# DEEPDIP-project/IncompressibleNavierStokes.jl

Measured on AMD Instinct MI355X. Metric: M lattice-cell updates/sec (RK4 step incl. Poisson), 3D TGV fp64, higher is better.
Workload: dtype f64; 1 GPU; TaylorGreenVortex3D 256^3 periodic fp64, RK44 + spectral Poisson, dt=0.001, Re=1e3; decomposition=single GPU, loop=timesteps_ (K steps, one native call)

## Files before the change

incompressiblenavierstokes.jl_amd/csrc/ins_flux128.hip:

```cpp
#include <algorithm>
#include <cstring>

#include "ins_internal.h"
#include "ins_wave64.h"
#include "ins_flux_common.h"

namespace {

template <typename T>
struct P2 {
  T a, b;
};
template <typename T>
__device__ __forceinline__ P2<T> ldb2(rsrc_t r, unsigned voff, unsigned soff);
template <>
__device__ __forceinline__ P2<double> ldb2<double>(rsrc_t r, unsigned voff, unsigned soff) {
  const v4u v = __builtin_amdgcn_raw_buffer_load_b128(r, voff, soff, 0);
  return {__hiloint2double((int)v.y, (int)v.x), __hiloint2double((int)v.w, (int)v.z)};
}
template <>
__device__ __forceinline__ P2<float> ldb2<float>(rsrc_t r, unsigned voff, unsigned soff) {
  const v2u v = __builtin_amdgcn_raw_buffer_load_b64(r, voff, soff, 0);
  return {__int_as_float((int)v.x), __int_as_float((int)v.y)};
}
// ... 6 lines not shown
  __builtin_amdgcn_raw_buffer_store_b128(v, r, voff, soff, 0);
}
__device__ __forceinline__ void stb2(rsrc_t r, unsigned voff, unsigned soff, float a, float b) {
  v2u v;
  v.x = (unsigned)__float_as_int(a);
  v.y = (unsigned)__float_as_int(b);
  __builtin_amdgcn_raw_buffer_store_b64(v, r, voff, soff, 0);
}

template <typename T, int R>
struct Plane2 {
  P2<T> v[3][R + 2];
  T h[3];
};

template <typename T, int R, int XW, bool FUSE, int CORR, int NW>
__global__ __launch_bounds__(64 * NW, (CORR && R == 2 && NW == 4 && sizeof(T) == 8) ? 1 : 2) void k_flux128(FluxArgs a) {
  constexpr unsigned EB = (unsigned)sizeof(T);
  constexpr int WC = 128;
  const T* const a_u = static_cast<const T*>(a.u);
  const T* const a_pI = static_cast<const T*>(a.pI);
  T* const a_F = static_cast<T*>(a.F);
  static_assert(R + 3 <= 8, "packed halo rows live in 8-lane groups");
  int txi, tyi, tzi;
  {
    const int nty_local = (a.nty + 7) >> 3;
    int seq = (int)(blockIdx.x >> 3);
    if (seq >= a.ntx * nty_local * a.ntz) return;
    txi = seq % a.ntx;
    seq /= a.ntx;
    tyi = (int)(blockIdx.x & 7) * nty_local + seq % nty_local;
    tzi = seq / nty_local;
// ... 87 lines not shown
      const T Wn = next_h(Wa, rdlane(C.h[2], 16 + rr));
      zprev[0][rr - 1].a = flux(C.v[0][rr].a, Nx.v[0][rr].a, Wa, Wb, Z.vo);
      zprev[0][rr - 1].b = flux(C.v[0][rr].b, Nx.v[0][rr].b, Wb, Wn, Z.vo);
      zprev[1][rr - 1].a = flux(C.v[1][rr].a, Nx.v[1][rr].a, Wa, C.v[2][rr + 1].a, Z.vo);
      zprev[1][rr - 1].b = flux(C.v[1][rr].b, Nx.v[1][rr].b, Wb, C.v[2][rr + 1].b, Z.vo);
      zprev[2][rr - 1].a = flux(Wa, Nx.v[2][rr].a, Wa, Nx.v[2][rr].a, Z.vs);
      zprev[2][rr - 1].b = flux(Wb, Nx.v[2][rr].b, Wb, Nx.v[2][rr].b, Z.vs);
    }
  };

  unsigned orow[R];
#pragma unroll
  for (int rr = 0; rr < R; ++rr) orow[rr] = (unsigned)((min(jb0 + rr, n1 - 1) + 1) * N0) * EB;
  const unsigned ocol = ucol;

  auto epi_load = [&](const Plane2<T, R>& C, int k, P2<T> (&sacc)[3][R]) {
    const long long pk = (long long)k * sz;
    if (a.epi.ustart) {
      const T* b = static_cast<const T*>((const void*)a.epi.ustart) + pk;
      const T c0 = (T)(1.0 + a.epi.c0m1);
#pragma unroll
      for (int c = 0; c < 3; ++c) {
        const rsrc_t rs = plane_rsrc(b + c * a.sc, ubytes);
#pragma unroll
        for (int rr = 0; rr < R; ++rr) {
          const P2<T> v = ldb2<T>(rs, ocol, orow[rr]);
          sacc[c][rr].a = c0 * v.a;
          sacc[c][rr].b = c0 * v.b;
        }
      }
    } else {
#pragma unroll
      for (int c = 0; c < 3; ++c)
#pragma unroll
        for (int rr = 0; rr < R; ++rr) sacc[c][rr] = C.v[c][rr + 1];
    }
    if (a.epi.self_in != 0.0) {
      const T cs = (T)a.epi.self_in;
      if (CORR) {
        const T* b = a_u + (long long)uplane(k) * sz;
#pragma unroll
// ... 21 lines not shown
      const T cq = (T)a.epi.coef[q];
#pragma unroll
      for (int c = 0; c < 3; ++c) {
        const rsrc_t rs = plane_rsrc(kq + c * a.sc, ubytes);
        P2<T> kv[R];
#pragma unroll
        for (int rr = 0; rr < R; ++rr) kv[rr] = ldb2<T>(rs, ocol, orow[rr]);
#pragma unroll
        for (int rr = 0; rr < R; ++rr) {
          sacc[c][rr].a += cq * kv[rr].a;
          sacc[c][rr].b += cq * kv[rr].b;
        }
      }
    }
  };
  auto emit = [&](int rr, int k, const P2<T>& fu, const P2<T>& fv, const P2<T>& fw, const P2<T>& s0, const P2<T>& s1, const P2<T>& s2) {
    const long long pk = (long long)k * sz;
    const int j = jb0 + rr - 1;
    if (xout && j < n1) {
      const unsigned rowb = orow[rr - 1], co = ocol;
      if (FUSE) {
        if (CORR && a.epi.ustart_out) {
          T* w = static_cast<T*>((void*)a.epi.ustart_out) + pk;
          stb2(plane_rsrc(w, ubytes), co, rowb, s0.a, s0.b);
          stb2(plane_rsrc(w + a.sc, ubytes), co, rowb, s1.a, s1.b);
          stb2(plane_rsrc(w + 2 * a.sc, ubytes), co, rowb, s2.a, s2.b);
        }
        T* o = static_cast<T*>((void*)a.epi.ustar) + pk;
        const T cs = (T)a.epi.coef_self;
        stb2(plane_rsrc(o, ubytes), co, rowb, s0.a + cs * fu.a, s0.b + cs * fu.b);
        stb2(plane_rsrc(o + a.sc, ubytes), co, rowb, s1.a + cs * fv.a, s1.b + cs * fv.b);
        stb2(plane_rsrc(o + 2 * a.sc, ubytes), co, rowb, s2.a + cs * fw.a, s2.b + cs * fw.b);
      }
      if (!FUSE || a.epi.write_k) {
        T* o = a_F + pk;
        stb2(plane_rsrc(o, ubytes), co, rowb, fu.a, fu.b);
        stb2(plane_rsrc(o + a.sc, ubytes), co, rowb, fv.a, fv.b);
        stb2(plane_rsrc(o + 2 * a.sc, ubytes), co, rowb, fw.a, fw.b);
      }
    }
  };

  auto body = [&](Plane2<T, R>& C, const Plane2<T, R>& Nx, int k, int kload) {
    const T* nb = a_u + (long long)uplane(kload) * sz;
    const rsrc_t n0r = plane_rsrc(nb, ubytes), n1r = plane_rsrc(nb + a.sc, ubytes), n2r = plane_rsrc(nb + 2 * a.sc, ubytes);
    const T ch0 = C.h[0], ch1 = C.h[1], ch2 = C.h[2];
    P2<T> sacc[3][FUSE ? R : 1];
    if constexpr (FUSE) epi_load(C, k, sacc);
    P2<T> fyu_o = {0, 0}, fyv_o = {0, 0}, fyw_o = {0, 0};
#pragma unroll
    for (int rr = 0; rr <= R; ++rr) {
      const T Ua = C.v[0][rr].a, Ub = C.v[0][rr].b, Va = C.v[1][rr].a, Vb = C.v[1][rr].b, Wa = C.v[2][rr].a, Wb = C.v[2][rr].b;
      const T Vn = next_h(Va, rdlane(ch1, 16 + rr));
      P2<T> fyu, fyv, fyw;
      fyu.a = flux(Ua, C.v[0][rr + 1].a, Va, Vb, Y.vo);
      fyu.b = flux(Ub, C.v[0][rr + 1].b, Vb, Vn, Y.vo);
      fyv.a = flux(Va, C.v[1][rr + 1].a, Va, C.v[1][rr + 1].a, Y.vs);
      fyv.b = flux(Vb, C.v[1][rr + 1].b, Vb, C.v[1][rr + 1].b, Y.vs);
      fyw.a = flux(Wa, C.v[2][rr + 1].a, Va, Nx.v[1][rr].a, Y.vo);
      fyw.b = flux(Wb, C.v[2][rr + 1].b, Vb, Nx.v[1][rr].b, Y.vo);
      if (rr >= 1) {
        const T Un = next_h(Ua, rdlane(ch0, 16 + rr)), Wn = next_h(Wa, rdlane(ch2, 16 + rr));
        const T fxu_a = flux(Ua, Ub, Ua, Ub, X.vs), fxu_b = flux(Ub, Un, Ub, Un, X.vs);
// ... 21 lines not shown
        zu.a = flux(Ua, Nx.v[0][rr].a, Wa, Wb, Z.vo);
        zu.b = flux(Ub, Nx.v[0][rr].b, Wb, Wn, Z.vo);
        zv.a = flux(Va, Nx.v[1][rr].a, Wa, C.v[2][rr + 1].a, Z.vo);
        zv.b = flux(Vb, Nx.v[1][rr].b, Wb, C.v[2][rr + 1].b, Z.vo);
        zw.a = flux(Wa, Nx.v[2][rr].a, Wa, Nx.v[2][rr].a, Z.vs);
        zw.b = flux(Wb, Nx.v[2][rr].b, Wb, Nx.v[2][rr].b, Z.vs);
        fu.a += (zu.a - zprev[0][rr - 1].a) * Z.ro;
        fu.b += (zu.b - zprev[0][rr - 1].b) * Z.ro;
        fv.a += (zv.a - zprev[1][rr - 1].a) * Z.ro;
        fv.b += (zv.b - zprev[1][rr - 1].b) * Z.ro;
        fw.a += (zw.a - zprev[2][rr - 1].a) * Z.rs;
        fw.b += (zw.b - zprev[2][rr - 1].b) * Z.rs;
        zprev[0][rr - 1] = zu;
        zprev[1][rr - 1] = zv;
        zprev[2][rr - 1] = zw;
        if constexpr (FUSE)
          emit(rr, k, fu, fv, fw, sacc[0][rr - 1], sacc[1][rr - 1], sacc[2][rr - 1]);
        else
          emit(rr, k, fu, fv, fw, fu, fu, fu);
      }
      fyu_o = fyu;
      fyv_o = fyv;
      fyw_o = fyw;
      C.v[0][rr] = ldb2<T>(n0r, ucol, urow[rr]);
      C.v[1][rr] = ldb2<T>(n1r, ucol, urow[rr]);
      C.v[2][rr] = ldb2<T>(n2r, ucol, urow[rr]);
    }
    C.v[0][R + 1] = ldb2<T>(n0r, ucol, urow[R + 1]);
    C.v[1][R + 1] = ldb2<T>(n1r, ucol, urow[R + 1]);
    C.v[2][R + 1] = ldb2<T>(n2r, ucol, urow[R + 1]);
    C.h[0] = ldb<T>(n0r, uhoff, 0);
// ... 38 lines not shown
      if (++k >= k1) break;
      if (a.bar) __builtin_amdgcn_s_barrier();
      correct(P1, Pb, Hb, Pa, Ha);
      load_p(Pb, Hb, min(k + 3, k1 + 1));
      body(P0, P1, k, min(k + 2, k1));
      if (++k >= k1) break;
    }
  }
}

template <typename T, int R, int XW, bool FUSE, int NW>
int launch_range(FluxArgs& a, int corr_mode, hipStream_t s) {
  const unsigned nb = (unsigned)(8LL * a.ntx * ((a.nty + 7) / 8) * a.ntz);
  if (nb == 0) return INS_OK;
  const dim3 block(64, NW, 1);
  if (corr_mode == 0)
    hipLaunchKernelGGL((k_flux128<T, R, XW, FUSE, 0, NW>), dim3(nb), block, 0, s, a);
  else if constexpr (FUSE) {
    if (corr_mode == 1)
      hipLaunchKernelGGL((k_flux128<T, R, XW, true, 1, NW>), dim3(nb), block, 0, s, a);
    else
      hipLaunchKernelGGL((k_flux128<T, R, XW, true, 2, NW>), dim3(nb), block, 0, s, a);
  } else {
    ins_set_error("in-kernel pressure correction needs the fused epilogue");
    return INS_ERR_UNSUPPORTED;
  }
  INS_LAUNCH_CHECK();
  return INS_OK;
}

// ... 118 lines not shown
```

incompressiblenavierstokes.jl_amd/csrc/ins_flux64.hip:

```cpp
#include <algorithm>
#include <cstdlib>
#include <cstring>

#include "ins_internal.h"
#include "ins_wave64.h"
#include "ins_flux_common.h"

namespace {

template <typename T, int R>
struct Plane {
  T v[3][R + 2];
  T h[3];
  T raw[3][R];
};

template <typename T, int R>
struct TExt {
  T t[R + 2];
  T th;
  T vm1;
};

template <typename T, int R, int XW, bool FUSE, int CORR, bool SKEL = false, int NW = 4, bool EXTRA = false>
__global__ __launch_bounds__(64 * NW, NW == 16 ? 4 : 2) void k_flux64(FluxArgs a) {
  constexpr unsigned EB = (unsigned)sizeof(T);
  const T* const a_u = static_cast<const T*>(a.u);
  const T* const a_pI = static_cast<const T*>(a.pI);
  T* const a_F = static_cast<T*>(a.F);
  static_assert(R + 2 + (CORR ? 1 : 0) <= 8, "packed halo rows live in 8-lane groups");
  int txi, tyi, tzi;
  {
    const int nty_local = (a.nty + 7) >> 3;
    int seq = (int)(blockIdx.x >> 3);
    if (seq >= a.ntx * nty_local * a.ntz) return;
    txi = seq % a.ntx;
    seq /= a.ntx;
    tyi = (int)(blockIdx.x & 7) * nty_local + seq % nty_local;
    tzi = seq / nty_local;
    if (tyi >= a.nty) return;
// ... 61 lines not shown
  auto load_text = [&](TExt<T, R>& E, int kk) {
    const long long po = (long long)uplane(kk) * sz;
    const rsrc_t rt = plane_rsrc(static_cast<const T*>((const void*)a.te.temp) + po, ubytes);
#pragma unroll
    for (int rr = 0; rr < R + 2; ++rr) E.t[rr] = ldb<T>(rt, ucol, urow[rr]);
    E.th = ldb<T>(rt, uhoff, 0);
    E.vm1 = ldb<T>(plane_rsrc(a_u + po + a.sc, ubytes), ucol, urowm1);
  };
  auto load_p = [&](T (&P)[R + 3], T& PH, int kk) {
    const rsrc_t rs = plane_rsrc(a_pI + (long long)(CORR == 2 ? min(kk, N2) : wrapi(kk - 1, n2)) * n0 * n1, qbytes);
#pragma unroll
    for (int rr = 0; rr < R + 3; ++rr) P[rr] = ldb<T>(rs, qcol, qrow[rr]);
    PH = ldb<T>(rs, qhoff, 0);
  };
  auto correct = [&](Plane<T, R>& P, const T (&Pc)[R + 3], T PHc, const T (&Pn)[R + 3], T PHn) {
    if (a.epi.self_in != 0.0) {
#pragma unroll
      for (int c = 0; c < 3; ++c)
#pragma unroll
        for (int rr = 0; rr < R; ++rr) P.raw[c][rr] = P.v[c][rr + 1];
    }
#pragma unroll
    for (int rr = 0; rr < R + 2; ++rr) {
      const T pc = Pc[rr];
      P.v[0][rr] -= (next_h(pc, rdlane(PHc, 16 + rr)) - pc) * X.gs;
      P.v[1][rr] -= (Pc[rr + 1] - pc) * Y.gs;
      P.v[2][rr] -= (Pn[rr] - pc) * Z.gs;
    }
    P.h[0] -= (dpp_old<0x108>(PHc, PHc) - PHc) * X.gs;
    P.h[1] -= (dpp_old<0x101>(PHc, PHc) - PHc) * Y.gs;
    P.h[2] -= (PHn - PHc) * Z.gs;
// ... 7 lines not shown
      zprev[0][rr - 1] = flux(C.v[0][rr], Nx.v[0][rr], Wc, next_h(Wc, rdlane(C.h[2], 16 + rr)), Z.vo);
      zprev[1][rr - 1] = flux(C.v[1][rr], Nx.v[1][rr], Wc, C.v[2][rr + 1], Z.vo);
      zprev[2][rr - 1] = flux(Wc, Nx.v[2][rr], Wc, Nx.v[2][rr], Z.vs);
    }
  };

  unsigned orow[R];
#pragma unroll
  for (int rr = 0; rr < R; ++rr) orow[rr] = (unsigned)((min(jb0 + rr, n1 - 1) + 1) * N0) * EB;
  const unsigned ocol = (unsigned)(min(ci, n0 - 1) + 1) * EB;

  T eacc[3][EXTRA ? R : 1];
  T gacc[EXTRA ? R : 1];
  T Pz[3][EXTRA ? R : 1];
  const T nux = X.vs * X.rs, nuy = Y.vs * Y.rs, nuz = Z.vs * Z.rs;
  auto epi_load = [&](const Plane<T, R>& C, int k, T (&sacc)[3][R]) {
    const long long pk = (long long)k * sz;
    if constexpr (EXTRA) {
      if (a.epi.extra) {
        const T* b = static_cast<const T*>((const void*)a.epi.extra) + pk;
#pragma unroll
        for (int c = 0; c < 3; ++c) {
          const rsrc_t rs = plane_rsrc(b + c * a.sc, ubytes);
#pragma unroll
          for (int rr = 0; rr < R; ++rr) eacc[c][rr] = ldb<T>(rs, ocol, orow[rr]);
        }
      } else {
#pragma unroll
        for (int c = 0; c < 3; ++c)
#pragma unroll
          for (int rr = 0; rr < R; ++rr) eacc[c][rr] = 0;
// ... 3 lines not shown
        const int gd = a.epi.gdir;
        const rsrc_t r0 = plane_rsrc(tb, ubytes), r1 = plane_rsrc(gd == 2 ? tb + sz : tb, ubytes);
        const unsigned dcol = gd == 0 ? EB : 0u, drow = gd == 1 ? (unsigned)N0 * EB : 0u;
#pragma unroll
        for (int rr = 0; rr < R; ++rr) gacc[rr] = (T)a.epi.ga2 * ((T)0.5 * (ldb<T>(r0, ocol, orow[rr]) + ldb<T>(r1, ocol + dcol, orow[rr] + drow)));
      }
    }
    const bool ntl = (a.nt & 8) != 0;
    if (a.epi.ustart) {
      const T* b = static_cast<const T*>((const void*)a.epi.ustart) + pk;
      const T c0 = (T)(1.0 + a.epi.c0m1);
#pragma unroll
      for (int c = 0; c < 3; ++c) {
        const rsrc_t rs = plane_rsrc(b + c * a.sc, ubytes);
#pragma unroll
        for (int rr = 0; rr < R; ++rr) sacc[c][rr] = c0 * (ntl ? ldb_aux<2>(rs, ocol, orow[rr], (T)0) : ldb<T>(rs, ocol, orow[rr]));
      }
    } else {
#pragma unroll
      for (int c = 0; c < 3; ++c)
#pragma unroll
        for (int rr = 0; rr < R; ++rr) sacc[c][rr] = C.v[c][rr + 1];
    }
    if (a.epi.self_in != 0.0) {
#pragma unroll
      for (int c = 0; c < 3; ++c)
#pragma unroll
        for (int rr = 0; rr < R; ++rr) sacc[c][rr] += (T)a.epi.self_in * (CORR ? C.raw[c][rr] : C.v[c][rr + 1]);
    }
    for (int q = 0; q < a.epi.n; ++q) {
      const T* kq = static_cast<const T*>((const void*)a.epi.k[q]) + pk;
// ... 18 lines not shown
      stb(r2, co, rowb, v2);
    } else if (snt == 1) {
      stb_aux<2>(r0, co, rowb, v0);
      stb_aux<2>(r1, co, rowb, v1);
      stb_aux<2>(r2, co, rowb, v2);
    } else if (snt == 2) {
      stb_aux<17>(r0, co, rowb, v0);
      stb_aux<17>(r1, co, rowb, v1);
      stb_aux<17>(r2, co, rowb, v2);
    } else {
      stb_aux<19>(r0, co, rowb, v0);
      stb_aux<19>(r1, co, rowb, v1);
      stb_aux<19>(r2, co, rowb, v2);
    }
  };
  auto emit = [&](int rr, int k, T fu, T fv, T fw, T s0, T s1, T s2) {
    const long long pk = (long long)k * sz;
    if constexpr (EXTRA) {
      fu += eacc[0][rr - 1];
      fv += eacc[1][rr - 1];
      fw += eacc[2][rr - 1];
      if (a.epi.gtemp) {
        const T gv = gacc[rr - 1];
        if (a.epi.gdir == 0) fu += gv;
        if (a.epi.gdir == 1) fv += gv;
        if (a.epi.gdir == 2) fw += gv;
      }
    }
    const int j = jb0 + rr - 1;
    if (xout && j < n1) {
      const unsigned rowb = orow[rr - 1], co = ocol;
      if (FUSE) {
        if (CORR && a.epi.ustart_out) {
          T* w = static_cast<T*>((void*)a.epi.ustart_out) + pk;
          stb(plane_rsrc(w, ubytes), co, rowb, s0);
          stb(plane_rsrc(w + a.sc, ubytes), co, rowb, s1);
          stb(plane_rsrc(w + 2 * a.sc, ubytes), co, rowb, s2);
        }
        T* o = static_cast<T*>((void*)a.epi.ustar) + pk;
        st3(o, co, rowb, s0 + (T)a.epi.coef_self * fu, s1 + (T)a.epi.coef_self * fv, s2 + (T)a.epi.coef_self * fw);
      }
      if (!FUSE || a.epi.write_k) st3(a_F + pk, co, rowb, fu, fv, fw);
    }
  };

  constexpr bool TMK = EXTRA && CORR == 0;
  T Tz[TMK ? R : 1];
  T wwprev[TMK ? R : 1];
  T PzV0 = 0;
  T hU_prev = 0;
  auto body = [&](Plane<T, R>& C, const Plane<T, R>& Nx, TExt<T, R>& CT, const TExt<T, R>& NT, int k, int kload) {
    const T* nb = a_u + (long long)uplane(kload) * sz;
    const rsrc_t n0r = plane_rsrc(nb, ubytes), n1r = plane_rsrc(nb + a.sc, ubytes), n2r = plane_rsrc(nb + 2 * a.sc, ubytes);
    const T ch0 = C.h[0], ch1 = C.h[1], ch2 = C.h[2];
    T sacc[3][R];
    if (FUSE) epi_load(C, k, sacc);
    const bool tm = TMK && a.tm;
    const rsrc_t ntr = plane_rsrc(static_cast<const T*>((const void*)a.te.temp) + (long long)uplane(kload) * sz, ubytes);
    T tacc[TMK ? R : 1];
    const T cth = CT.th;
    if constexpr (TMK) {
      if (tm) {
        const long long pk = (long long)k * sz;
        const rsrc_t rs0 = plane_rsrc(static_cast<const T*>((const void*)a.te.tempstart) + pk, ubytes);
#pragma unroll
        for (int rr = 0; rr < R; ++rr) tacc[rr] = ldb<T>(rs0, ocol, orow[rr]);
        for (int q = 0; q < a.te.n; ++q) {
          const rsrc_t rq = plane_rsrc(static_cast<const T*>((const void*)a.te.k[q]) + pk, ubytes);
#pragma unroll
          for (int rr = 0; rr < R; ++rr) tacc[rr] += (T)a.te.coef[q] * ldb<T>(rq, ocol, orow[rr]);
        }
// ... 80 lines not shown
              const T kt = cd + dd;
              if (xout && j < n1) {
                const long long pk = (long long)k * sz;
                if (a.te.ktemp_out) stb(plane_rsrc(static_cast<T*>((void*)a.te.ktemp_out) + pk, ubytes), ocol, orow[rr - 1], kt);
                stb(plane_rsrc(static_cast<T*>((void*)a.te.temp_out) + pk, ubytes), ocol, orow[rr - 1], tacc[rr - 1] + (T)a.te.c_self * kt);
              }
              wv_o = wv;
              wwprev[rr - 1] = ww;
              Tz[rr - 1] = Tc;
            }
          }
          Pz[0][rr - 1] = Uc;
          Pz[1][rr - 1] = Vc;
          Pz[2][rr - 1] = Wc;
        }
        emit(rr, k, fu, fv, fw, FUSE ? sacc[0][rr - 1] : (T)0, FUSE ? sacc[1][rr - 1] : (T)0, FUSE ? sacc[2][rr - 1] : (T)0);
      }
      fyu_o = fyu;
      fyv_o = fyv;
      fyw_o = fyw;
      if constexpr (TMK) {
        if (tm) {
          if (rr == 0) {
            const T Vp = prev_h(Vc, rdlane(ch1, 0));
            wv_o = jb0 > 0 ? Vc * ((Vn + Vp - 2 * Vc) * nux + (C.v[1][1] + CT.vm1 - 2 * Vc) * nuy + (Nx.v[1][0] + PzV0 - 2 * Vc) * nuz) : (T)0;
            PzV0 = Vc;
          }
          To = CT.t[rr];
          CT.t[rr] = ldb<T>(ntr, ucol, urow[rr]);
        }
      }
// ... 104 lines not shown
#define g_lds ((int)ins_opt(OPT_INS_FLUX64_LDS))
#define g_skel ((int)ins_opt(OPT_INS_FLUX64_SKEL))

template <typename T, int R, int XW, bool FUSE, int NW>
int launch_range(const ins_grid* G, FluxArgs& a, int corr_mode, hipStream_t s) {
  const unsigned nb = (unsigned)(8LL * a.ntx * ((a.nty + 7) / 8) * a.ntz);
  if (nb == 0) return INS_OK;
  const dim3 block(64, NW, 1);
  if constexpr (NW <= 8 && R == 4 && sizeof(T) == 8) {
    if (g_skel && corr_mode == 0) {
      hipLaunchKernelGGL((k_flux64<T, R, XW, FUSE, 0, true, NW>), dim3(nb), block, (size_t)g_lds, s, a);
      INS_LAUNCH_CHECK();
      return INS_OK;
    }
  }
  if (a.tm && corr_mode != 0) {
    ins_set_error("temperature stage inside the stage kernel: no in-kernel pressure correction");
    return INS_ERR_UNSUPPORTED;
  }
  if (a.epi.extra || a.epi.gtemp || a.epi.wout || a.tm) {
    if constexpr (FUSE && R == 2 && NW == 4 && sizeof(T) == 8) {
      if (corr_mode == 0) {
        hipLaunchKernelGGL((k_flux64<T, R, XW, true, 0, false, NW, true>), dim3(nb), block, (size_t)g_lds, s, a);
        INS_LAUNCH_CHECK();
        return INS_OK;
      }
      if (corr_mode == 1) {
        hipLaunchKernelGGL((k_flux64<T, R, XW, true, 1, false, NW, true>), dim3(nb), block, (size_t)g_lds, s, a);
        INS_LAUNCH_CHECK();
        return INS_OK;
// ... 46 lines not shown

extern "C" void ins_tune_flux64(int disable, int rows, int rows_corr, int zchunk, int xw, int skel, int burst_unused, int lds) {
  if (disable >= 0) ins_set_option("INS_DISABLE_FLUX64", disable);
  if (rows >= 0) ins_set_option("INS_FLUX64_ROWS", rows);
  if (rows_corr >= 0) ins_set_option("INS_FLUX64_ROWS_CORR", rows_corr);
  if (zchunk >= 0) ins_set_option("INS_FLUX64_ZC", zchunk);
  if (xw >= 0) ins_set_option("INS_FLUX64_XW", xw);
  if (skel >= 0) ins_set_option("INS_FLUX64_SKEL", skel);
  (void)burst_unused;
  if (lds >= 0) ins_set_option("INS_FLUX64_LDS", lds);
}

bool ins_flux64_supported(const ins_grid* G) {
  const GridDev& g = G->g;
  return !g_disable && g.D == 3 && G->all_dof && G->uniform_exact && g.N[0] - 2 >= 66 && g.N[1] - 2 >= 8 && g.N[2] - 2 >= 4;
}

template <typename T>
static int flux64_dispatch(const ins_grid* G, double visc, const T* u, T* F, const RkEpi* epi, const T* pI, int corr_mode, hipStream_t s, int part) {
  const GridDev& g = G->g;
  FluxArgs a;
  memset(&a, 0, sizeof(a));
  a.u = u;
  a.pI = pI;
  a.F = F;
  a.sc = g.sc;
  a.N0 = g.N[0];
  a.N1 = g.N[1];
  a.N2 = g.N[2];
  const int n2 = g.N[2] - 2;
// ... 109 lines not shown
```

incompressiblenavierstokes.jl_amd/csrc/ins_flux_common.h:

```cpp
#pragma once
#include "ins_internal.h"

namespace {

struct Dir {
  double vs, vo;
  double rs, ro;
  double gs;
};
template <typename T>
struct DirT {
  T vs, vo, rs, ro, gs;
  __device__ DirT(const Dir& d) : vs((T)d.vs), vo((T)d.vo), rs((T)d.rs), ro((T)d.ro), gs((T)d.gs) {}
};

struct FluxArgs {
  const void* u;
  const void* pI;
  void* F;
  long long sc;
  int N0, N1, N2;
  int zc, ntx, nty, ntz;
  int k_lo, k_hi, kB;
  int nt;
  int bar;
  Dir X, Y, Z;
  RkEpi epi;
  int tm;
  TempEpi te;
};

template <typename T>
__device__ __forceinline__ T flux(T uc, T up, T ub0, T ub1, T vd4) {
  return (up - uc) * vd4 - (uc + up) * (ub0 + ub1);
}

static Dir make_dir(const ins_grid* G, int d, double visc) {
  const double dxu = G->desc.dxu[d][1], dx1 = G->desc.dx[d][1], dx2 = G->desc.dx[d][2];
  Dir r;
  r.vs = 4.0 * (visc * (dx2 > 2 * INS_EPS ? 1.0 / dx2 : 0.0));
  r.vo = 4.0 * (visc * (dxu > 2 * INS_EPS ? 1.0 / dxu : 0.0));
  r.gs = 1.0 / dxu;
  r.rs = 0.25 * r.gs;
  r.ro = 0.25 * (1.0 / dx1);
  return r;
}

}
```

incompressiblenavierstokes.jl_amd/csrc/ins_internal.h:

```cpp
#pragma once

#include <hip/hip_runtime.h>
#include <hipfft/hipfft.h>

#include <cstdint>
#include <cstdio>
#include <cstring>
#include <string>
#include <vector>

#include "ins_hip.h"

#define INS_EPS 2.220446049250313e-16
#define INS_MAX_STAGES 16

void ins_set_error(const char* fmt, ...);

#define INS_HIP_TRY(expr)                                                                   \
  do {                                                                                      \
    hipError_t _e = (expr);                                                                 \
    if (_e != hipSuccess) {                                                                 \
      ins_set_error("%s:%d: %s -> %s", __FILE__, __LINE__, #expr, hipGetErrorString(_e));   \
      return INS_ERR_HIP;                                                                   \
    }                                                                                       \
// ... 69 lines not shown
  X(INS_FLUX64_LDS)              \
  X(INS_FLUX64_SKEL)             \
  X(INS_FLUX64_NW)               \
  X(INS_FLUX64_NT)               \
  X(INS_FLUX64_NOBAR)            \
  X(INS_FLUX64_MINTILES)         \
  X(INS_FLUX64_XW_CORR)          \
  X(INS_UNIFORM_BITWISE)         \
  X(INS_PHAT_DENSE)              \
  X(INS_DISABLE_FDM_FUSED)       \
  X(INS_DISABLE_FDM_FOLD)        \
  X(INS_DISABLE_FDM_UNFOLD4)     \
  X(INS_DISABLE_FDM_FOLDFUSE)    \
  X(INS_DISABLE_INKERNEL_CORR)   \
  X(INS_RK_KEEP_K)               \
  X(INS_DISABLE_EXT_FUSED)       \
  X(INS_EXT_TEMP_SPLIT)          \
  X(INS_DISABLE_FUSED_RK)        \
  X(INS_DISABLE_STEP_CHAIN)      \
  X(INS_DISABLE_STEP_GRAPH)      \
  X(INS_DISABLE_LINE3)           \
  X(INS_DISABLE_XYFUSED)         \
  X(INS_DISABLE_CORR2D)          \
  X(INS_SPECTRUM_ROCFFT)         \
  X(INS_X_SKEL)                  \
  X(INS_LINE3_TK)                \
  X(INS_LINE3_WGS)               \
  X(INS_STEP_GRAPH)              \
  X(INS_ZSOLVE_SKEL)             \
  X(INS_ZSOLVE_TK)               \
// ... 141 lines not shown
struct Rec {
  double vs, vo, a0, b0, a1, b1, a2, b2, rs, ro, pad[6];
};

struct RkEpi {
  int n;
  int write_k;
  double coef[INS_MAX_STAGES + 1];
  const double* k[INS_MAX_STAGES + 1];
  double coef_self;
  double self_in;
  double c0m1;
  const double* ustart;
  double* ustar;
  double* ustart_out;
  const double* extra;
  const double* gtemp;
  double ga2;
  int gdir;
  double* wout;
  const struct TempEpi* tstage;
};

struct TempEpi {
  const double* temp;
  const double* tempstart;
  double* temp_out;
  double* ktemp_out;
  int n;
  double coef[INS_MAX_STAGES];
// ... 90 lines not shown
```

incompressiblenavierstokes.jl_amd/csrc/ins_rk.hip:

```cpp
#include <cstdlib>

#include "ins_internal.h"


int ins_k_momentum_generic(const ins_grid* G, double visc, const double* u, double* F, hipStream_t s);
int ins_k_momentum_fast3d(const ins_grid* G, double visc, const double* u, double* F, hipStream_t s);
int ins_k_momentum_fast3d_opts(const ins_grid* G, double visc, const double* u, double* F, bool zero_shell, hipStream_t s);
bool ins_fast3d_supported(const ins_grid* G);
bool ins_flux64_supported(const ins_grid* G);

int ins_k_momentum_rk_fused(const ins_grid* G, double visc, const double* u_in, double* k_out, const RkEpi& epi, hipStream_t s);
int ins_k_project_periodic_fused(const ins_grid* G, ins_poisson* ps, double* u, double* p, bool keep_p, hipStream_t s, double* uout = nullptr);

int ins_k_momentum(const ins_grid* G, double visc, const double* u, double* F, hipStream_t s) {
  if (ins_fast3d_supported(G)) return ins_k_momentum_fast3d(G, visc, u, F, s);
  return ins_k_momentum_generic(G, visc, u, F, s);
}

namespace {

struct Combine {
  int n;
  double coef[INS_MAX_STAGES + 1];
  const double* k[INS_MAX_STAGES + 1];
// ... 37 lines not shown
static int combine_n(long long nvec, const double* base, double* out, int nterms, const double* coefs, const double* const* ks, void* stream) {
  INS_REQUIRE(nterms >= 0 && nterms <= INS_MAX_STAGES + 1 && (nterms == 0 || (coefs && ks)), "bad stage terms");
  Combine cb;
  cb.n = 0;
  for (int q = 0; q < nterms; ++q) {
    if (coefs[q] == 0.0) continue;
    INS_REQUIRE(ks[q], "null stage field");
    cb.coef[cb.n] = coefs[q];
    cb.k[cb.n] = ks[q];
    ++cb.n;
  }
  const unsigned nblk = (unsigned)std::min<long long>((nvec / 2 + 255) / 256, 8192);
  hipLaunchKernelGGL(k_combine, dim3(nblk), dim3(256), 0, as_stream(stream), nvec, base, out, cb);
  INS_LAUNCH_CHECK();
  return INS_OK;
}

static void step_graph_free(ins_rk* rk);
bool ins_k_spectral_own3d(const ins_poisson* ps);

extern "C" int ins_rk_create(const ins_grid_t* G, ins_poisson_t* ps, int nstage, const double* A, const double* c, ins_rk_t** out) {
  INS_REQUIRE(G && ps && A && c && out, "null argument");
  INS_REQUIRE(ps->grid == G, "psolver was created for a different grid");
  INS_REQUIRE(nstage >= 1 && nstage <= INS_MAX_STAGES, "unsupported number of stages");
  for (int i = 0; i < nstage; ++i)
    for (int j = i + 1; j < nstage; ++j) INS_REQUIRE(A[i * nstage + j] == 0.0, "shifted tableau must be lower triangular (explicit method)");
  ins_rk* rk = new ins_rk();
  rk->grid = G;
  rk->ps = ps;
  rk->nstage = nstage;
// ... 78 lines not shown
  const int ns = rk->nstage;
  const size_t vbytes = (size_t)G->ncell * 3 * sizeof(double);
  for (int b = 0; b < 2; ++b)
    if (!rk->ub[b]) {
      INS_HIP_TRY(hipMalloc(&rk->ub[b], vbytes));
      INS_HIP_TRY(hipMemsetAsync(rk->ub[b], 0, vbytes, s));
    }
  int rc;
  const bool raw_in = chain & 1, raw_out = chain & 2;
  if (!raw_in && (rc = ins_k_apply_bc_u(G, u, 0, nullptr, s))) return rc;
  const bool no_corr = ins_opt(OPT_INS_DISABLE_INKERNEL_CORR) != 0;
  const bool inkernel = !no_corr && G->uniform_exact && ns > 1 && G->g.N[0] >= 8 && G->g.N[1] >= 8 && G->g.N[2] >= 8;
  const bool keep_k = ins_opt(OPT_INS_RK_KEEP_K) != 0;
  bool vbasis = inkernel && !keep_k;
  for (int i = 0; vbasis && i < ns; ++i) vbasis = rk->A[i * ns + i] != 0.0;
  if (vbasis && (int)rk->vb.size() < ns - 1) {
    rk->vb.resize(ns - 1, nullptr);
    for (int m = 0; m < ns - 1; ++m)
      if (!rk->vb[m]) {
        if (m < 2 && rk->ub[m]) {
          rk->vb[m] = rk->ub[m];
          continue;
        }
        INS_HIP_TRY(hipMalloc(&rk->vb[m], vbytes));
        INS_HIP_TRY(hipMemsetAsync(rk->vb[m], 0, vbytes, s));
      }
  }
  const double* in = u;
  for (int i = 0; i < ns; ++i) {
    double* out = (i == ns - 1 && ns > 1) ? u : (vbasis ? rk->vb[i] : rk->ub[i & 1]);
    RkEpi epi;
    memset(&epi, 0, sizeof(epi));
    if (vbasis) {
      double beta[INS_MAX_STAGES];
      for (int m = i - 1; m >= 0; --m) {
        double v = rk->A[i * ns + m];
        for (int j = m + 1; j < i; ++j) v -= beta[j] * rk->A[j * ns + m];
        beta[m] = v / rk->A[m * ns + m];
      }
      const bool flux64 = ins_flux64_supported(G);
      for (int m = 0; m < i; ++m) {
        if (beta[m] == 0.0) continue;
        epi.c0m1 -= beta[m];
        if (m == i - 1 && flux64) {
          epi.self_in = beta[m];
          continue;
        }
        epi.coef[epi.n] = beta[m];
        epi.k[epi.n] = rk->vb[m];
        ++epi.n;
      }
    } else {
      for (int j = 0; j < i; ++j) {
        const double coef = dt * rk->A[i * ns + j];
        if (coef == 0.0) continue;
        epi.coef[epi.n] = coef;
        epi.k[epi.n] = rk->ku[j];
        ++epi.n;
      }
      for (int i2 = i + 1; i2 < ns; ++i2)
        if (rk->A[i2 * ns + i] != 0.0) epi.write_k = 1;
    }
    if (rk->force) {
      double cf = dt * rk->A[i * ns + i];
      if (!vbasis)
        for (int j = 0; j < i; ++j) cf += dt * rk->A[i * ns + j];
      epi.coef[epi.n] = cf;
      epi.k[epi.n] = rk->force;
      ++epi.n;
    }
    epi.coef_self = dt * rk->A[i * ns + i];
    epi.ustart = (i == 0) ? nullptr : (raw_in ? rk->ustart : u);
    epi.ustar = out;
    if (i == 0 && raw_in) epi.ustart_out = rk->ustart;
    hipEvent_t e0 = nullptr, e1 = nullptr;
    if (rk->profiling) {
      INS_HIP_TRY(hipEventCreate(&e0));
      INS_HIP_TRY(hipEventCreate(&e1));
      INS_HIP_TRY(hipEventRecord(e0, s));
    }
    rc = (inkernel && (i > 0 || raw_in)) ? ins_k_momentum_rk_fused_corr(G, visc, in, rk->ps->pI, rk->ku[i], epi, s)
                             : ins_k_momentum_rk_fused(G, visc, in, rk->ku[i], epi, s);
    if (rc) return rc;
    if (rk->profiling) {
      INS_HIP_TRY(hipEventRecord(e1, s));
      rk->prof_events.push_back(e0);
      rk->prof_events.push_back(e1);
// ... 374 lines not shown
```

Before: 6716 M cell-updates/s.

## Carry a pre-combined RK stage basis buffer through the fused stage kernel

Adds a stage planner that, for later RK stages combining several earlier stage velocities, has an earlier stage kernel write an extra pre-combined carry buffer (ustart and raw inputs weighted, plus the new stage value). The later stage then reads that one buffer in place of ustart and multiple stage buffers, cutting the number of full-field reads in the memory-bound stage kernel. This costs an extra full-field store in the producing stage and adds planner-driven buffer assignment. Unsupported configurations fall back or error.

New measurement: 6477 M cell-updates/s. -3.5%, worse.

```diff
diff --git a/incompressiblenavierstokes.jl_amd/csrc/ins_flux128.hip b/incompressiblenavierstokes.jl_amd/csrc/ins_flux128.hip
--- a/incompressiblenavierstokes.jl_amd/csrc/ins_flux128.hip
+++ b/incompressiblenavierstokes.jl_amd/csrc/ins_flux128.hip
@@ -4,6 +4,8 @@
 #include "ins_internal.h"
 #include "ins_wave64.h"
 #include "ins_flux_common.h"
+
+extern long long g_ins_carry_launches[2];
 
 namespace {
 
@@ -44,8 +46,9 @@
   T h[3];
 };
 
-template <typename T, int R, int XW, bool FUSE, int CORR, int NW>
+template <typename T, int R, int XW, bool FUSE, int CORR, int NW, bool CARRY = false>
 __global__ __launch_bounds__(64 * NW, (CORR && R == 2 && NW == 4 && sizeof(T) == 8) ? 1 : 2) void k_flux128(FluxArgs a) {
+  static_assert(!CARRY || (FUSE && CORR == 1), "the carry store belongs to the correcting fused form");
   constexpr unsigned EB = (unsigned)sizeof(T);
   constexpr int WC = 128;
   const T* const a_u = static_cast<const T*>(a.u);
@@ -163,7 +166,7 @@
   for (int rr = 0; rr < R; ++rr) orow[rr] = (unsigned)((min(jb0 + rr, n1 - 1) + 1) * N0) * EB;
   const unsigned ocol = ucol;
 
-  auto epi_load = [&](const Plane2<T, R>& C, int k, P2<T> (&sacc)[3][R]) {
+  auto epi_load = [&](const Plane2<T, R>& C, int k, P2<T> (&sacc)[3][R], P2<T> (&wacc)[3][CARRY ? R : 1]) {
     const long long pk = (long long)k * sz;
     if (a.epi.ustart) {
       const T* b = static_cast<const T*>((const void*)a.epi.ustart) + pk;
@@ -174,6 +177,12 @@
 #pragma unroll
         for (int rr = 0; rr < R; ++rr) {
           const P2<T> v = ldb2<T>(rs, ocol, orow[rr]);
+          if constexpr (CARRY) {
+            P2<T> rw = {0, 0};
+            if (a.epi.carry_raw != 0.0) rw = ldb2<T>(plane_rsrc(a_u + (long long)uplane(k) * sz + c * a.sc, ubytes), ucol, urow[rr + 1]);
+            wacc[c][rr].a = rk_carry_begin((T)a.epi.carry_u, v.a, (T)a.epi.carry_raw, rw.a);
+            wacc[c][rr].b = rk_carry_begin((T)a.epi.carry_u, v.b, (T)a.epi.carry_raw, rw.b);
+          }
           sacc[c][rr].a = c0 * v.a;
           sacc[c][rr].b = c0 * v.b;
         }
@@ -225,7 +234,8 @@
       }
     }
   };
-  auto emit = [&](int rr, int k, const P2<T>& fu, const P2<T>& fv, const P2<T>& fw, const P2<T>& s0, const P2<T>& s1, const P2<T>& s2) {
+  auto emit = [&](int rr, int k, const P2<T>& fu, const P2<T>& fv, const P2<T>& fw, const P2<T>& s0, const P2<T>& s1, const P2<T>& s2,
+                  const P2<T>* wc = nullptr) {
     const long long pk = (long long)k * sz;
     const int j = jb0 + rr - 1;
     if (xout && j < n1) {
@@ -239,9 +249,18 @@
         }
         T* o = static_cast<T*>((void*)a.epi.ustar) + pk;
         const T cs = (T)a.epi.coef_self;
-        stb2(plane_rsrc(o, ubytes), co, rowb, s0.a + cs * fu.a, s0.b + cs * fu.b);
-        stb2(plane_rsrc(o + a.sc, ubytes), co, rowb, s1.a + cs * fv.a, s1.b + cs * fv.b);
-        stb2(plane_rsrc(o + 2 * a.sc, ubytes), co, rowb, s2.a + cs * fw.a, s2.b + cs * fw.b);
+        const P2<T> v0 = {s0.a + cs * fu.a, s0.b + cs * fu.b}, v1 = {s1.a + cs * fv.a, s1.b + cs * fv.b}, v2 = {s2.a + cs * fw.a, s2.b + cs * fw.b};
+        stb2(plane_rsrc(o, ubytes), co, rowb, v0.a, v0.b);
+        stb2(plane_rsrc(o + a.sc, ubytes), co, rowb, v1.a, v1.b);
+        stb2(plane_rsrc(o + 2 * a.sc, ubytes), co, rowb, v2.a, v2.b);
+        if constexpr (CARRY) {
+          T* w = static_cast<T*>((void*)a.epi.carry_out) + pk;
+          const bool any = a.epi.carry_u != 0.0 || a.epi.carry_raw != 0.0;
+          const T cn = (T)a.epi.carry_new;
+          stb2(plane_rsrc(w, ubytes), co, rowb, rk_carry_end(wc[0].a, any, cn, v0.a), rk_carry_end(wc[0].b, any, cn, v0.b));
+          stb2(plane_rsrc(w + a.sc, ubytes), co, rowb, rk_carry_end(wc[1].a, any, cn, v1.a), rk_carry_end(wc[1].b, any, cn, v1.b));
+          stb2(plane_rsrc(w + 2 * a.sc, ubytes), co, rowb, rk_carry_end(wc[2].a, any, cn, v2.a), rk_carry_end(wc[2].b, any, cn, v2.b));
+        }
       }
       if (!FUSE || a.epi.write_k) {
         T* o = a_F + pk;
@@ -257,7 +276,8 @@
     const rsrc_t n0r = plane_rsrc(nb, ubytes), n1r = plane_rsrc(nb + a.sc, ubytes), n2r = plane_rsrc(nb + 2 * a.sc, ubytes);
     const T ch0 = C.h[0], ch1 = C.h[1], ch2 = C.h[2];
     P2<T> sacc[3][FUSE ? R : 1];
-    if constexpr (FUSE) epi_load(C, k, sacc);
+    P2<T> wacc[3][CARRY ? R : 1];
+    if constexpr (FUSE) epi_load(C, k, sacc, wacc);
     P2<T> fyu_o = {0, 0}, fyv_o = {0, 0}, fyw_o = {0, 0};
 #pragma unroll
     for (int rr = 0; rr <= R; ++rr) {
@@ -309,7 +329,10 @@
         zprev[0][rr - 1] = zu;
         zprev[1][rr - 1] = zv;
         zprev[2][rr - 1] = zw;
-        if constexpr (FUSE)
+        if constexpr (CARRY) {
+          const P2<T> wc[3] = {wacc[0][rr - 1], wacc[1][rr - 1], wacc[2][rr - 1]};
+          emit(rr, k, fu, fv, fw, sacc[0][rr - 1], sacc[1][rr - 1], sacc[2][rr - 1], wc);
+        } else if constexpr (FUSE)
           emit(rr, k, fu, fv, fw, sacc[0][rr - 1], sacc[1][rr - 1], sacc[2][rr - 1]);
         else
           emit(rr, k, fu, fv, fw, fu, fu, fu);
@@ -378,6 +401,18 @@
   const unsigned nb = (unsigned)(8LL * a.ntx * ((a.nty + 7) / 8) * a.ntz);
   if (nb == 0) return INS_OK;
   const dim3 block(64, NW, 1);
+  if (a.epi.carry_out) {
+    if constexpr (FUSE && R == 1 && sizeof(T) == 8) {
+      if (corr_mode == 1) {
+        hipLaunchKernelGGL((k_flux128<T, R, XW, true, 1, NW, true>), dim3(nb), block, 0, s, a);
+        INS_LAUNCH_CHECK();
+        ++g_ins_carry_launches[1];
+        return INS_OK;
+      }
+    }
+    ins_set_error("carried stage combination: fp64 correcting stage kernel of a periodic box with 1 row of pairs per lane only (ins_rk_carry_supported)");
+    return INS_ERR_UNSUPPORTED;
+  }
   if (corr_mode == 0)
     hipLaunchKernelGGL((k_flux128<T, R, XW, FUSE, 0, NW>), dim3(nb), block, 0, s, a);
   else if constexpr (FUSE) {
diff --git a/incompressiblenavierstokes.jl_amd/csrc/ins_flux64.hip b/incompressiblenavierstokes.jl_amd/csrc/ins_flux64.hip
--- a/incompressiblenavierstokes.jl_amd/csrc/ins_flux64.hip
+++ b/incompressiblenavierstokes.jl_amd/csrc/ins_flux64.hip
@@ -5,6 +5,9 @@
 #include "ins_internal.h"
 #include "ins_wave64.h"
 #include "ins_flux_common.h"
+
+long long g_ins_carry_launches[2] = {0, 0};
+extern "C" long long ins_dbg_rk_carry_launches(int two_columns) { return g_ins_carry_launches[two_columns ? 1 : 0]; }
 
 namespace {
 
@@ -22,8 +25,9 @@
   T vm1;
 };
 
-template <typename T, int R, int XW, bool FUSE, int CORR, bool SKEL = false, int NW = 4, bool EXTRA = false>
+template <typename T, int R, int XW, bool FUSE, int CORR, bool SKEL = false, int NW = 4, bool EXTRA = false, bool CARRY = false>
 __global__ __launch_bounds__(64 * NW, NW == 16 ? 4 : 2) void k_flux64(FluxArgs a) {
+  static_assert(!CARRY || (FUSE && CORR == 1 && !SKEL && !EXTRA), "the carry store belongs to the correcting fused form");
   constexpr unsigned EB = (unsigned)sizeof(T);
   const T* const a_u = static_cast<const T*>(a.u);
   const T* const a_pI = static_cast<const T*>(a.pI);
@@ -115,7 +119,7 @@
     PH = ldb<T>(rs, qhoff, 0);
   };
   auto correct = [&](Plane<T, R>& P, const T (&Pc)[R + 3], T PHc, const T (&Pn)[R + 3], T PHn) {
-    if (a.epi.self_in != 0.0) {
+    if (a.epi.self_in != 0.0 || (CARRY && a.epi.carry_raw != 0.0)) {
 #pragma unroll
       for (int c = 0; c < 3; ++c)
 #pragma unroll
@@ -153,7 +157,7 @@
   T gacc[EXTRA ? R : 1];
   T Pz[3][EXTRA ? R : 1];
   const T nux = X.vs * X.rs, nuy = Y.vs * Y.rs, nuz = Z.vs * Z.rs;
-  auto epi_load = [&](const Plane<T, R>& C, int k, T (&sacc)[3][R]) {
+  auto epi_load = [&](const Plane<T, R>& C, int k, T (&sacc)[3][R], T (&wacc)[3][CARRY ? R : 1]) {
     const long long pk = (long long)k * sz;
     if constexpr (EXTRA) {
       if (a.epi.extra) {
@@ -187,7 +191,15 @@
       for (int c = 0; c < 3; ++c) {
         const rsrc_t rs = plane_rsrc(b + c * a.sc, ubytes);
 #pragma unroll
-        for (int rr = 0; rr < R; ++rr) sacc[c][rr] = c0 * (ntl ? ldb_aux<2>(rs, ocol, orow[rr], (T)0) : ldb<T>(rs, ocol, orow[rr]));
+        for (int rr = 0; rr < R; ++rr) {
+          if constexpr (CARRY) {
+            const T us = ntl ? ldb_aux<2>(rs, ocol, orow[rr], (T)0) : ldb<T>(rs, ocol, orow[rr]);
+            wacc[c][rr] = rk_carry_begin((T)a.epi.carry_u, us, (T)a.epi.carry_raw, C.raw[c][rr]);
+            sacc[c][rr] = c0 * us;
+          } else {
+            sacc[c][rr] = c0 * (ntl ? ldb_aux<2>(rs, ocol, orow[rr], (T)0) : ldb<T>(rs, ocol, orow[rr]));
+          }
+        }
       }
     } else {
 #pragma unroll
@@ -236,7 +248,7 @@
       stb_aux<19>(r2, co, rowb, v2);
     }
   };
-  auto emit = [&](int rr, int k, T fu, T fv, T fw, T s0, T s1, T s2) {
+  auto emit = [&](int rr, int k, T fu, T fv, T fw, T s0, T s1, T s2, T w0 = 0, T w1 = 0, T w2 = 0) {
     const long long pk = (long long)k * sz;
     if constexpr (EXTRA) {
       fu += eacc[0][rr - 1];
@@ -260,7 +272,13 @@
           stb(plane_rsrc(w + 2 * a.sc, ubytes), co, rowb, s2);
         }
         T* o = static_cast<T*>((void*)a.epi.ustar) + pk;
-        st3(o, co, rowb, s0 + (T)a.epi.coef_self * fu, s1 + (T)a.epi.coef_self * fv, s2 + (T)a.epi.coef_self * fw);
+        const T v0 = s0 + (T)a.epi.coef_self * fu, v1 = s1 + (T)a.epi.coef_self * fv, v2 = s2 + (T)a.epi.coef_self * fw;
+        st3(o, co, rowb, v0, v1, v2);
+        if constexpr (CARRY) {
+          const bool any = a.epi.carry_u != 0.0 || a.epi.carry_raw != 0.0;
+          const T cn = (T)a.epi.carry_new;
+          st3(static_cast<T*>((void*)a.epi.carry_out) + pk, co, rowb, rk_carry_end(w0, any, cn, v0), rk_carry_end(w1, any, cn, v1), rk_carry_end(w2, any, cn, v2));
+        }
       }
       if (!FUSE || a.epi.write_k) st3(a_F + pk, co, rowb, fu, fv, fw);
     }
@@ -276,7 +294,8 @@
     const rsrc_t n0r = plane_rsrc(nb, ubytes), n1r = plane_rsrc(nb + a.sc, ubytes), n2r = plane_rsrc(nb + 2 * a.sc, ubytes);
     const T ch0 = C.h[0], ch1 = C.h[1], ch2 = C.h[2];
     T sacc[3][R];
-    if (FUSE) epi_load(C, k, sacc);
+    T wacc[3][CARRY ? R : 1];
+    if (FUSE) epi_load(C, k, sacc, wacc);
     const bool tm = TMK && a.tm;
     const rsrc_t ntr = plane_rsrc(static_cast<const T*>((const void*)a.te.temp) + (long long)uplane(kload) * sz, ubytes);
     T tacc[TMK ? R : 1];
@@ -387,7 +406,10 @@
           Pz[1][rr - 1] = Vc;
           Pz[2][rr - 1] = Wc;
         }
-        emit(rr, k, fu, fv, fw, FUSE ? sacc[0][rr - 1] : (T)0, FUSE ? sacc[1][rr - 1] : (T)0, FUSE ? sacc[2][rr - 1] : (T)0);
+        if constexpr (CARRY)
+          emit(rr, k, fu, fv, fw, sacc[0][rr - 1], sacc[1][rr - 1], sacc[2][rr - 1], wacc[0][rr - 1], wacc[1][rr - 1], wacc[2][rr - 1]);
+        else
+          emit(rr, k, fu, fv, fw, FUSE ? sacc[0][rr - 1] : (T)0, FUSE ? sacc[1][rr - 1] : (T)0, FUSE ? sacc[2][rr - 1] : (T)0);
       }
       fyu_o = fyu;
       fyv_o = fyv;
@@ -522,6 +544,18 @@
       return INS_OK;
     }
   }
+  if (a.epi.carry_out) {
+    if constexpr (FUSE && R == 2 && NW <= 8 && sizeof(T) == 8) {
+      if (corr_mode == 1 && !(a.epi.extra || a.epi.gtemp || a.epi.wout || a.tm)) {
+        hipLaunchKernelGGL((k_flux64<T, R, XW, true, 1, false, NW, false, true>), dim3(nb), block, (size_t)g_lds, s, a);
+        INS_LAUNCH_CHECK();
+        ++g_ins_carry_launches[0];
+        return INS_OK;
+      }
+    }
+    ins_set_error("carried stage combination: fp64 correcting stage kernel of a periodic box with 2 rows per lane only (ins_rk_carry_supported)");
+    return INS_ERR_UNSUPPORTED;
+  }
   if (a.tm && corr_mode != 0) {
     ins_set_error("temperature stage inside the stage kernel: no in-kernel pressure correction");
     return INS_ERR_UNSUPPORTED;
@@ -598,6 +632,13 @@
 bool ins_flux64_supported(const ins_grid* G) {
   const GridDev& g = G->g;
   return !g_disable && g.D == 3 && G->all_dof && G->uniform_exact && g.N[0] - 2 >= 66 && g.N[1] - 2 >= 8 && g.N[2] - 2 >= 4;
+}
+
+bool ins_flux128_supported(const ins_grid* G, const RkEpi* epi, int corr_mode, bool f32);
+bool ins_rk_carry_supported(const ins_grid* G) {
+  if (!ins_flux64_supported(G) || g_skel || ins_opt(OPT_INS_FLUX64_NW) == 16) return false;
+  if (ins_flux128_supported(G, nullptr, 1, false)) return ins_opt(OPT_INS_FLUX128_ROWS_CORR) != 2;
+  return g_rows_corr <= 2;
 }
 
 template <typename T>
diff --git a/incompressiblenavierstokes.jl_amd/csrc/ins_flux_common.h b/incompressiblenavierstokes.jl_amd/csrc/ins_flux_common.h
--- a/incompressiblenavierstokes.jl_amd/csrc/ins_flux_common.h
+++ b/incompressiblenavierstokes.jl_amd/csrc/ins_flux_common.h
@@ -35,6 +35,20 @@
   return (up - uc) * vd4 - (uc + up) * (ub0 + ub1);
 }
 
+__device__ __forceinline__ double fma_t(double a, double b, double c) { return __builtin_fma(a, b, c); }
+__device__ __forceinline__ float fma_t(float a, float b, float c) { return __builtin_fmaf(a, b, c); }
+template <typename T>
+__device__ __forceinline__ T rk_carry_begin(T cu, T us, T cr, T raw) {
+  T w = 0;
+  if (cu != (T)0) w = cu * us;
+  if (cr != (T)0) w = cu != (T)0 ? fma_t(cr, raw, w) : cr * raw;
+  return w;
+}
+template <typename T>
+__device__ __forceinline__ T rk_carry_end(T w, bool any, T cn, T ustar) {
+  return any ? fma_t(cn, ustar, w) : cn * ustar;
+}
+
 static Dir make_dir(const ins_grid* G, int d, double visc) {
   const double dxu = G->desc.dxu[d][1], dx1 = G->desc.dx[d][1], dx2 = G->desc.dx[d][2];
   Dir r;
diff --git a/incompressiblenavierstokes.jl_amd/csrc/ins_internal.h b/incompressiblenavierstokes.jl_amd/csrc/ins_internal.h
--- a/incompressiblenavierstokes.jl_amd/csrc/ins_internal.h
+++ b/incompressiblenavierstokes.jl_amd/csrc/ins_internal.h
@@ -107,6 +107,7 @@
   X(INS_DISABLE_FDM_FOLDFUSE)    \
   X(INS_DISABLE_INKERNEL_CORR)   \
   X(INS_RK_KEEP_K)               \
+  X(INS_DISABLE_RK_CARRY)        \
   X(INS_DISABLE_EXT_FUSED)       \
   X(INS_EXT_TEMP_SPLIT)          \
   X(INS_DISABLE_FUSED_RK)        \
@@ -278,6 +279,8 @@
   const double* ustart;
   double* ustar;
   double* ustart_out;
+  double* carry_out;
+  double carry_u, carry_raw, carry_new;
   const double* extra;
   const double* gtemp;
   double ga2;
diff --git a/incompressiblenavierstokes.jl_amd/csrc/ins_rk.hip b/incompressiblenavierstokes.jl_amd/csrc/ins_rk.hip
--- a/incompressiblenavierstokes.jl_amd/csrc/ins_rk.hip
+++ b/incompressiblenavierstokes.jl_amd/csrc/ins_rk.hip
@@ -1,6 +1,7 @@
 #include <cstdlib>
 
 #include "ins_internal.h"
+#include "ins_rk_plan.h"
 
 
 int ins_k_momentum_generic(const ins_grid* G, double visc, const double* u, double* F, hipStream_t s);
@@ -8,6 +9,7 @@
 int ins_k_momentum_fast3d_opts(const ins_grid* G, double visc, const double* u, double* F, bool zero_shell, hipStream_t s);
 bool ins_fast3d_supported(const ins_grid* G);
 bool ins_flux64_supported(const ins_grid* G);
+bool ins_rk_carry_supported(const ins_grid* G);
 
 int ins_k_momentum_rk_fused(const ins_grid* G, double visc, const double* u_in, double* k_out, const RkEpi& epi, hipStream_t s);
 int ins_k_project_periodic_fused(const ins_grid* G, ins_poisson* ps, double* u, double* p, bool keep_p, hipStream_t s, double* uout = nullptr);
@@ -75,6 +77,28 @@
   hipLaunchKernelGGL(k_combine, dim3(nblk), dim3(256), 0, as_stream(stream), nvec, base, out, cb);
   INS_LAUNCH_CHECK();
   return INS_OK;
+}
+
+extern "C" int ins_dbg_rk_plan(int ns, const double* A, int self_in_ok, int carry, double* out, int cap) {
+  InsRkPlan P;
+  if (!out || ins_rk_plan(ns, A, self_in_ok, carry, &P) != 0) return -1;
+  const int rec = 13 + 4 * ns, total = 3 + ns * rec;
+  if (cap < total) return -1;
+  out[0] = P.ns, out[1] = P.nbuf, out[2] = P.ncarry;
+  for (int i = 0; i < ns; ++i) {
+    const InsRkStagePlan& S = P.st[i];
+    double* o = out + 3 + i * rec;
+    const double head[13] = {S.c0m1, S.c0, (double)S.base_src, S.base_coef, S.self_in, (double)S.n, (double)S.out_buf, (double)S.carry_for, (double)S.carry_buf,
+                             S.carry_u, S.carry_raw, S.carry_new, (double)S.carry_from};
+    for (int q = 0; q < 13; ++q) o[q] = head[q];
+    for (int m = 0; m < ns; ++m) {
+      o[13 + m] = S.beta[m];
+      o[13 + ns + m] = m < S.n ? S.src_stage[m] : -1;
+      o[13 + 2 * ns + m] = m < S.n ? S.src[m] : -1;
+      o[13 + 3 * ns + m] = m < S.n ? S.coef[m] : 0.0;
+    }
+  }
+  return total;
 }
 
 static void step_graph_free(ins_rk* rk);
@@ -183,6 +207,15 @@
   const bool keep_k = ins_opt(OPT_INS_RK_KEEP_K) != 0;
   bool vbasis = inkernel && !keep_k;
   for (int i = 0; vbasis && i < ns; ++i) vbasis = rk->A[i * ns + i] != 0.0;
+  InsRkPlan plan;
+  if (vbasis) {
+    const bool flux64 = ins_flux64_supported(G);
+    const bool carry = flux64 && !ins_opt(OPT_INS_DISABLE_RK_CARRY) && !rk->ext && ins_rk_carry_supported(G);
+    if (ins_rk_plan(ns, rk->A.data(), flux64, carry, &plan) != 0 || plan.nbuf > ns - 1) {
+      ins_set_error("stage plan of the stage-velocity basis failed");
+      return INS_ERR_INVALID;
+    }
+  }
   if (vbasis && (int)rk->vb.size() < ns - 1) {
     rk->vb.resize(ns - 1, nullptr);
     for (int m = 0; m < ns - 1; ++m)
@@ -197,27 +230,28 @@
   }
   const double* in = u;
   for (int i = 0; i < ns; ++i) {
-    double* out = (i == ns - 1 && ns > 1) ? u : (vbasis ? rk->vb[i] : rk->ub[i & 1]);
+    double* out = (i == ns - 1 && ns > 1) ? u : (vbasis ? rk->vb[plan.st[i].out_buf] : rk->ub[i & 1]);
     RkEpi epi;
     memset(&epi, 0, sizeof(epi));
+    const double* carried = nullptr;
     if (vbasis) {
-      double beta[INS_MAX_STAGES];
-      for (int m = i - 1; m >= 0; --m) {
-        double v = rk->A[i * ns + m];
-        for (int j = m + 1; j < i; ++j) v -= beta[j] * rk->A[j * ns + m];
-        beta[m] = v / rk->A[m * ns + m];
-      }
-      const bool flux64 = ins_flux64_supported(G);
-      for (int m = 0; m < i; ++m) {
-        if (beta[m] == 0.0) continue;
-        epi.c0m1 -= beta[m];
-        if (m == i - 1 && flux64) {
-          epi.self_in = beta[m];
-          continue;
-        }
-        epi.coef[epi.n] = beta[m];
-        epi.k[epi.n] = rk->vb[m];
+      const InsRkStagePlan& S = plan.st[i];
+      epi.self_in = S.self_in;
+      for (int q = 0; q < S.n; ++q) {
+        epi.coef[epi.n] = S.coef[q];
+        epi.k[epi.n] = rk->vb[S.src[q]];
         ++epi.n;
+      }
+      if (S.carry_from >= 0) {
+        carried = rk->vb[S.base_src];
+      } else {
+        epi.c0m1 = S.c0m1;
+      }
+      if (S.carry_for >= 0) {
+        epi.carry_out = rk->vb[S.carry_buf];
+        epi.carry_u = S.carry_u;
+        epi.carry_raw = S.carry_raw;
+        epi.carry_new = S.carry_new;
       }
     } else {
       for (int j = 0; j < i; ++j) {
@@ -239,7 +273,7 @@
       ++epi.n;
     }
     epi.coef_self = dt * rk->A[i * ns + i];
-    epi.ustart = (i == 0) ? nullptr : (raw_in ? rk->ustart : u);
+    epi.ustart = (i == 0) ? nullptr : (carried ? carried : (raw_in ? rk->ustart : u));
     epi.ustar = out;
     if (i == 0 && raw_in) epi.ustart_out = rk->ustart;
     hipEvent_t e0 = nullptr, e1 = nullptr;
diff --git a/incompressiblenavierstokes.jl_amd/csrc/ins_rk_plan.h b/incompressiblenavierstokes.jl_amd/csrc/ins_rk_plan.h
--- /dev/null
+++ b/incompressiblenavierstokes.jl_amd/csrc/ins_rk_plan.h
@@ -0,0 +1,132 @@
+#pragma once
+
+#ifndef INS_MAX_STAGES
+#define INS_MAX_STAGES 16
+#endif
+
+enum { INS_RK_SRC_USTART = -1 };
+
+struct InsRkStagePlan {
+  double beta[INS_MAX_STAGES];
+  double c0m1, c0;
+  int base_src;
+  double base_coef;
+  double self_in;
+  int n;
+  int src[INS_MAX_STAGES];
+  int src_stage[INS_MAX_STAGES];
+  double coef[INS_MAX_STAGES];
+  int out_buf;
+  int carry_for;
+  int carry_buf;
+  double carry_u, carry_raw, carry_new;
+  int carry_from;
+};
+
+struct InsRkPlan {
+  int ns;
+  int nbuf;
+  int ncarry;
+  InsRkStagePlan st[INS_MAX_STAGES];
+};
+
+static inline int ins_rk_plan(int ns, const double* A, int self_in_ok, int carry, InsRkPlan* P) {
+  if (!A || !P || ns < 1 || ns > INS_MAX_STAGES) return -1;
+  for (int i = 0; i < ns; ++i)
+    if (A[i * ns + i] == 0.0) return -1;
+  for (int pass = 0; pass < 2; ++pass) {
+    P->ns = ns;
+    P->nbuf = 0;
+    P->ncarry = 0;
+    for (int i = 0; i < ns; ++i) {
+      InsRkStagePlan& S = P->st[i];
+      for (int m = 0; m < INS_MAX_STAGES; ++m) S.beta[m] = 0.0;
+      for (int m = i - 1; m >= 0; --m) {
+        double v = A[i * ns + m];
+        for (int j = m + 1; j < i; ++j) v -= S.beta[j] * A[j * ns + m];
+        S.beta[m] = v / A[m * ns + m];
+      }
+      double c0m1 = 0.0;
+      for (int m = 0; m < i; ++m)
+        if (S.beta[m] != 0.0) c0m1 -= S.beta[m];
+      S.c0m1 = c0m1;
+      S.c0 = 1.0 + c0m1;
+      S.base_src = INS_RK_SRC_USTART;
+      S.base_coef = S.c0;
+      S.self_in = 0.0;
+      S.n = 0;
+      S.out_buf = -1;
+      S.carry_for = S.carry_from = -1;
+      S.carry_buf = -1;
+      S.carry_u = S.carry_raw = S.carry_new = 0.0;
+    }
+    int mem_from[INS_MAX_STAGES];
+    for (int i = 0; i < ns; ++i) mem_from[i] = 0;
+    if (carry && pass == 0 && self_in_ok) {
+      for (int i = 2; i < ns; ++i) {
+        InsRkStagePlan& S = P->st[i];
+        int nmem = S.c0 != 0.0 ? 1 : 0, mstar = -1;
+        for (int m = 0; m < i - 1; ++m)
+          if (S.beta[m] != 0.0) {
+            ++nmem;
+            mstar = m;
+          }
+        if (nmem < 2 || mstar < 1) continue;
+        bool legal = P->st[mstar].carry_for < 0 && P->st[mstar].carry_from < 0;
+        for (int m = 0; m < mstar - 1; ++m)
+          if (S.beta[m] != 0.0) legal = false;
+        if (!legal) continue;
+        InsRkStagePlan& Q = P->st[mstar];
+        Q.carry_for = i;
+        Q.carry_u = S.c0;
+        Q.carry_raw = S.beta[mstar - 1];
+        Q.carry_new = S.beta[mstar];
+        S.carry_from = mstar;
+        S.base_coef = 1.0;
+        mem_from[i] = i - 1;
+        ++P->ncarry;
+      }
+    }
+    for (int i = 0; i < ns; ++i) {
+      InsRkStagePlan& S = P->st[i];
+      for (int m = 0; m < i; ++m) {
+        if (S.beta[m] == 0.0) continue;
+        if (m == i - 1 && self_in_ok) {
+          S.self_in = S.beta[m];
+          continue;
+        }
+        if (m < mem_from[i]) continue;
+        S.src_stage[S.n] = m;
+        S.coef[S.n] = S.beta[m];
+        ++S.n;
+      }
+    }
+    int last_read[2 * INS_MAX_STAGES];
+    int vbuf[INS_MAX_STAGES];
+    auto take = [&](int stage, int last) {
+      int b = 0;
+      while (b < P->nbuf && last_read[b] >= stage) ++b;
+      if (b == P->nbuf) ++P->nbuf;
+      last_read[b] = last;
+      return b;
+    };
+    for (int i = 0; i < ns; ++i) {
+      InsRkStagePlan& S = P->st[i];
+      if (i < ns - 1) {
+        int last = i + 1;
+        for (int j = i + 2; j < ns; ++j)
+          for (int q = 0; q < P->st[j].n; ++q)
+            if (P->st[j].src_stage[q] == i) last = j;
+        vbuf[i] = S.out_buf = take(i, last);
+      }
+      if (S.carry_for >= 0) {
+        S.carry_buf = take(i, S.carry_for);
+        P->st[S.carry_for].base_src = S.carry_buf;
+      }
+    }
+    for (int i = 0; i < ns; ++i)
+      for (int q = 0; q < P->st[i].n; ++q) P->st[i].src[q] = vbuf[P->st[i].src_stage[q]];
+    if (P->ncarry == 0 || P->nbuf <= (ns > 1 ? ns - 1 : 1)) break;
+  }
+  return 0;
+}
```
